# akashsengupta1997/STRAPS-3DHumanShapePose

Hardware: AMD Instinct MI355X
Metric: bodies/sec (higher is better)
Workload: dtype fp32 (encoder convolutions as exact bf16x3 operand splits (six bf16 products per term); in-step SMPL blend contraction and skinning as 3-product fp16 splits (fp16x3_lbs: 22-bit operands); fp32 accumulate throughout)

## Files before the change

include/straps_hip.h:

```cpp
#ifndef STRAPS_HIP_H
#define STRAPS_HIP_H

#include <stddef.h>
#include <stdint.h>

#ifdef __cplusplus
extern "C" {
#endif

#define STRAPS_ABI_VERSION 12

#define STRAPS_OK 0
#define STRAPS_EINVAL 1
#define STRAPS_EHIP 2
#define STRAPS_EUNSUPPORTED 3

int straps_abi_version(void);
int straps_selftest_mfma_peak(const float* seed512, float* out, int blocks, int iters, void* stream);
int straps_selftest_mfma_bf16(float* out, unsigned long long* clk2, int blocks, int iters, void* stream);
int straps_selftest_mfma_bf16_dense(float* out, unsigned long long* clk2, int blocks, int iters, int data, void* stream);
const char* straps_last_error(void);
int straps_device_count(void);
int straps_wall_clock_khz(void);
int straps_set_clock_accumulator(unsigned long long* acc2);
// ... 187 lines not shown
                         int cin, int cout, int kh, int kw, int stride, int pad, int tile_cfg, void* stream);
int straps_conv_dgrad_x3(const unsigned short* dy3, long long dy_plane_stride,
                         const unsigned short* w3_crsk, long long w_plane_stride,
                         const float* addend, float* dx_nhwc, int batch, int h, int w, int cin,
                         int cout, int kh, int kw, int stride, int pad, int tile_cfg, void* stream);
int straps_bn_apply_x3(const float* raw, const float* scale, const float* shift, const float* residual,
                       int relu, float* y, unsigned short* y_planes, long long plane_stride,
                       long long rows, int c, void* stream);
int straps_bn_relu_maxpool_fwd_x3(const float* raw, const float* scale, const float* shift,
                                  float* y_pool, uint8_t* idx, unsigned short* y_planes,
                                  long long plane_stride, int batch, int h, int w, int c, void* stream);
int straps_bn_bwd_x3(const float* dy, const float* yact, const float* raw, const float* save_mean,
                     const float* save_invstd, const float* gamma, const float* mask_scale,
                     const float* mask_shift, float* dgamma, float* dbeta, float* draw, float* dz_out,
                     unsigned short* draw_planes, long long plane_stride, void* workspace,
                     long long rows, int c, int accumulate, void* stream);
int straps_conv_dgrad_x3_bn_blocks(int batch, int h, int w, int cin, int cout, int kh, int kw, int stride,
                                   int pad, int tile_cfg);
int straps_conv_dgrad_x3_bn(const unsigned short* dy3, long long dy_plane_stride,
                            const unsigned short* w3_crsk, long long w_plane_stride, const float* addend,
                            float* dx_nhwc, int batch, int h, int w, int cin, int cout, int kh, int kw,
                            int stride, int pad, int tile_cfg, const float* bn_raw, const float* bn_out,
                            const float* bn_mask_scale, const float* bn_mask_shift, const float* bn_mean,
                            const float* bn_invstd, double* bn_partials, void* stream);
int straps_bn_bwd_finish_x3(const float* dy, const float* yact, const float* raw, const float* save_mean,
                            const float* save_invstd, const float* gamma, const float* mask_scale,
                            const float* mask_shift, float* dgamma, float* dbeta, float* draw, float* dz_out,
                            unsigned short* draw_planes, long long plane_stride, const double* partials,
                            int nblk, void* workspace, long long rows, int c, int accumulate, void* stream);
int straps_bn_apply_bits_x3(const float* raw, const float* scale, const float* shift, const float* residual, float* y,
                            unsigned short* y_planes, long long plane_stride, unsigned* relu_bits, long long rows,
                            int c, void* stream);
int straps_bn_bwd_bits_x3(const float* dy, const unsigned* relu_bits, const float* raw, const float* save_mean,
                          const float* save_invstd, const float* gamma, float* dgamma, float* dbeta, float* draw,
                          unsigned short* draw_planes, long long plane_stride, void* workspace, long long rows, int c,
                          int accumulate, void* stream);
int straps_bn_bwd_finish_bits_x3(const float* dy, const unsigned* relu_bits, const float* raw, const float* save_mean,
                                 const float* save_invstd, const float* gamma, float* dgamma, float* dbeta, float* draw,
                                 unsigned short* draw_planes, long long plane_stride, const double* partials, int nblk,
                                 void* workspace, long long rows, int c, int accumulate, void* stream);
int straps_conv_dgrad_x3_bits(const unsigned short* dy3, long long dy_plane_stride, const unsigned short* w3_crsk,
                              long long w_plane_stride, const float* addend, float* dx_nhwc, int batch, int h, int w,
                              int cin, int cout, int kh, int kw, int stride, int pad, int tile_cfg,
                              const unsigned* addend_bits, void* stream);
int straps_conv_dgrad_x3_bn_bits(const unsigned short* dy3, long long dy_plane_stride,
                                 const unsigned short* w3_crsk, long long w_plane_stride, const float* addend,
                                 float* dx_nhwc, int batch, int h, int w, int cin, int cout, int kh, int kw,
                                 int stride, int pad, int tile_cfg, const float* bn_raw, const float* bn_out,
                                 const float* bn_mask_scale, const float* bn_mask_shift, const float* bn_mean,
                                 const float* bn_invstd, double* bn_partials, const unsigned* addend_bits,
                                 const unsigned* bn_out_bits, void* stream);
int straps_conv_wgrad_x3_on_planes(int batch, int h, int w, int cin, int cout, int kh, int kw,
                                   int stride, int pad);
int straps_conv_wgrad_x3(const float* x_nhwc, const float* dy_nhwc, const unsigned short* x3,
                         long long x_plane_stride, const unsigned short* dy3, long long dy_plane_stride,
                         float* dw_oihw, void* workspace, int batch, int h, int w, int cin, int cout,
                         int kh, int kw, int stride, int pad, int accumulate, void* stream);


size_t straps_conv_wgrad_workspace_bytes(int batch, int h, int w, int cin, int cout, int kh,
                                         int kw, int stride, int pad);
int straps_conv_wgrad(const float* x_nhwc, const float* dy_nhwc, float* dw_oihw, void* workspace,
                      int batch, int h, int w, int cin, int cout, int kh, int kw, int stride,
                      int pad, int accumulate, void* stream);
size_t straps_stem_wgrad_workspace_bytes(int batch, int cin, int h, int w);
int straps_stem_wgrad(const float* x_nchw, const float* dy_nhwc, float* dw_oihw, void* workspace,
                      const uint32_t* nzmask , int batch, int cin,
                      int h, int w, int accumulate, void* stream);
#define STRAPS_STEM_DGRAD_MAX_CIN 64
size_t straps_stem_dgrad_weight_floats(int cin);
int straps_pack_stem_dgrad_weight(const float* w_oihw, float* w_pk, int cin, void* stream);
int straps_stem_dgrad(const float* dy_nhwc, const float* w_pk, float* dx_nchw, int batch, int cin, int h, int w,
                      int accumulate, void* stream);
int straps_bn_bwd_blocks(long long rows, int c);
size_t straps_bn_bwd_workspace_bytes(long long rows, int c);
int straps_bn_bwd(const float* dy, const float* yact, const float* raw, const float* save_mean,
                  const float* save_invstd, const float* gamma, const float* mask_scale,
                  const float* mask_shift, float* dgamma, float* dbeta, float* draw, float* dz_out,
                  void* workspace, long long rows, int c, int accumulate, void* stream);
int straps_bn_relu_maxpool_fwd(const float* raw_nhwc, const float* scale, const float* shift,
                               float* y_pool_nhwc, uint8_t* idx, int batch, int h, int w, int c,
                               void* stream);
int straps_bn_bwd_pooled(const float* dy_pool_nhwc, const uint8_t* idx, const float* raw,
                         const float* save_mean, const float* save_invstd, const float* gamma,
                         const float* mask_scale, const float* mask_shift, float* dgamma, float* dbeta,
                         float* draw, void* workspace, int batch, int h, int w, int c, int accumulate,
                         void* stream);
size_t straps_stem_tiles(int batch, int in_h, int in_w);
int straps_stem_tile_activity(const uint32_t* nzmask, uint8_t* tile_active, int batch, int cin, int in_h,
                              int in_w, void* stream);
int straps_bn_bwd_pooled_sparse(const float* dy_pool_nhwc, const uint8_t* idx, const float* raw,
                                const float* save_mean, const float* save_invstd, const float* gamma,
                                const float* mask_scale, const float* mask_shift, float* dgamma,
                                float* dbeta, float* draw, void* workspace, int batch, int h, int w, int c,
                                int accumulate, const uint8_t* tile_active, void* stream);
int straps_maxpool_fwd_idx(const float* x_nhwc, float* y_nhwc, uint8_t* idx, int batch, int h,
                           int w, int c, void* stream);
int straps_maxpool_bwd(const float* dy_nhwc, const uint8_t* idx, float* dx_nhwc, int batch, int h,
                       int w, int c, void* stream);
int straps_gap_bwd(const float* dfeat, float* dx_nhwc, int batch, int hw, int c, void* stream);
int straps_masked_copy(const float* x, int ldx, const float* mask, int ldmask, float* y, int ldy,
                       int m, int n, int accumulate, void* stream);
int straps_rot6d_bwd(const float* x6, long long ld, int per_row, const float* drot, float* dx6,
                     long long ldd, long long rows, void* stream);

int straps_build_proxy_input(const float* seg, const float* joints2d, float* out_nchw, int batch,
// ... 165 lines not shown
```

straps-3dhumanshapepose_amd/csrc/backward.hip:

```cpp
#include "common.h"
#include <stdlib.h>

namespace {

struct WgradP {
    const float* x;
    const float* dy;
    float* part;
    int B, H, W, Cin, Cout, R, S, stride, pad, Ho, Wo;
    int M, rows_per_split, ct, it;
};

__device__ __attribute__((aligned(16))) float k_zero16w[4] = {0.f, 0.f, 0.f, 0.f};

template <int BCO, int BCI>
__global__ __launch_bounds__(256) void conv_wgrad_kernel(WgradP p) {
    constexpr int STG = 32 * (BCO + BCI);
    constexpr int LPD = BCO / 4, PWD = 64 / LPD, RDD = 8 / PWD;
    constexpr int LPX = BCI / 4, PWX = 64 / LPX, RDX = 8 / PWX;
    constexpr int MI = BCO / 64, NI = BCI / 64;
    extern __shared__ __attribute__((aligned(16))) float smem[];
    const int tid = threadIdx.x, lane = tid & 63, wave = tid >> 6;
    const int wave_u = __builtin_amdgcn_readfirstlane(wave);
    const int wm = wave >> 1, wn = wave & 1;
// ... 404 lines not shown
            for (int c = 0; c < NI; ++c) {
                const int c4 = wn * (BCI / 2) + c * 32 + ch16 * 16 + (tt & 3) * 4;
                fx[ks][rd][c] = px * BCI + (((c4 >> 5) ^ seg_swz<BCI>(px)) << 5) + (c4 & 31);
            }
        }
    constexpr int TA[6] = {1, 0, 2, 0, 1, 0};
    constexpr int TB[6] = {1, 2, 0, 1, 0, 0};
    constexpr int DPS = 3 * (RDD + RDX);
    static_assert(DPS * (NST - 2) <= 63, "vmcnt range");
    int stage = 0;
    for (int st = 0; st < nsteps; ++st) {
        const int ahead = nsteps - 1 - st;
        if (NST >= 4 && ahead >= 2) asm volatile("s_waitcnt vmcnt(%0)" ::"n"(DPS * (NST >= 4 ? 2 : 0)) : "memory");
        else if (NST >= 3 && ahead >= 1) asm volatile("s_waitcnt vmcnt(%0)" ::"n"(DPS * (NST >= 3 ? 1 : 0)) : "memory");
        else asm volatile("s_waitcnt vmcnt(0)" ::: "memory");
        __builtin_amdgcn_s_barrier();
        asm volatile("" ::: "memory");
        if (st + NST - 1 < nsteps) dma_step(stage == 0 ? NST - 1 : stage - 1);
        const u16* D = smem + stage * STG;
        const u16* X = D + 3 * PLD;
        stage = stage + 1 == NST ? 0 : stage + 1;
        __builtin_amdgcn_s_setprio(1);
#pragma unroll
        for (int ks = 0; ks < 2; ++ks) {
            bf16x8w av[MI][3], bv[NI][3];
#pragma unroll
            for (int pl = 0; pl < 3; ++pl) {
#pragma unroll
                for (int a = 0; a < MI; ++a) av[a][pl] = tr_frag(D + pl * PLD + fd[ks][0][a], D + pl * PLD + fd[ks][1][a]);
#pragma unroll
                for (int c = 0; c < NI; ++c) bv[c][pl] = tr_frag(X + pl * PLX + fx[ks][0][c], X + pl * PLX + fx[ks][1][c]);
            }
#pragma unroll
            for (int e = 0; e < 6; ++e)
#pragma unroll
                for (int a = 0; a < MI; ++a)
#pragma unroll
                    for (int c = 0; c < NI; ++c)
                        acc[a][c] = __builtin_amdgcn_mfma_f32_32x32x16_bf16(av[a][TA[e]], bv[c][TB[e]], acc[a][c], 0, 0, 0);
        }
        __builtin_amdgcn_s_setprio(0);
    }
    const int i = lane & 31;
    const long long RS = (long long)p.R * p.S;
    float* o = p.part + (long long)split * p.Cout * RS * p.Cin;
#pragma unroll
    for (int a = 0; a < MI; ++a)
#pragma unroll
        for (int c = 0; c < NI; ++c)
#pragma unroll
            for (int q = 0; q < 16; ++q) {
                const int co = co0 + wm * (BCO / 2) + a * 32 + mfma_row(q, lane);
                o[((long long)co * RS + tap) * p.Cin + ci0 + wn * (BCI / 2) + c * 32 + i] = acc[a][c][q];
            }
}

template <int NG, int CP, int ABL = 0>
__global__ __launch_bounds__(256 * NG) void conv_wgrad3x3_x3_kernel(Wgrad3XP p) {
    constexpr int DPX = CP, XPX = CP == 32 ? 128 : 136;
    constexpr int STAGE = 3 * (DPX + XPX) * 64;
    constexpr int DR = CP / 32, XR = (XPX + 31) / 32;
    constexpr int KSG = CP / 16 / NG;
    static_assert(CP % (16 * NG) == 0, "chunk / group mismatch");
    extern __shared__ __attribute__((aligned(16))) float smem_f[];
    u16* smem = reinterpret_cast<u16*>(smem_f);
    const int pw = p.cw + 2;
    const int npatch = (p.rpc + 2) * pw;
    const int tid = threadIdx.x, lane = tid & 63, wave = (tid >> 6) & 3;
    const int grp = NG > 1 ? __builtin_amdgcn_readfirstlane(tid >> 8) : 0;
    const int wave_u = __builtin_amdgcn_readfirstlane(wave);
    const int wm = wave >> 1, wn = wave & 1;
    const int itile = blockIdx.x % p.it, ctile = blockIdx.x / p.it;
    const int co0 = ctile * 64, ci0 = itile * 64;
    const int cbeg = blockIdx.y * p.chunks_per_split;
    const int cend = min(cbeg + p.chunks_per_split, p.nchunks);
    const u16* zsrc = reinterpret_cast<const u16*>(k_zero16x);
    asm volatile("" : "+s"(zsrc));

    const int lp = (tid & 255) >> 3, ls = tid & 7;
    const int d_g = ls ^ (((lp >> 1) & 1) << 2);
    long long d_off[DR];
#pragma unroll
    for (int q = 0; q < DR; ++q) {
        const int px = lp + 32 * q;
        d_off[q] = ((long long)((co0 >> 5) + (d_g >> 2)) * p.rows + (px >> p.cw_log2) * p.W + (px & (p.cw - 1))) * 32 + (d_g & 3) * 8;
    }
    int x_pr[XR], x_pc[XR];
    long long x_g[XR];
#pragma unroll
    for (int q = 0; q < XR; ++q) {
        const int pp = lp + 32 * q;
        x_pr[q] = pp / pw - 1;
        x_pc[q] = pp - (x_pr[q] + 1) * pw - 1;
        const int g = ls ^ (((pp >> 1) & 1) << 2);
        x_g[q] = (long long)((ci0 >> 5) + (g >> 2)) * p.rows * 32 + (g & 3) * 8;
    }
    auto dma_chunk = [&](int c, int stage) {
        const int per_img = p.chunk_rows_per_img * p.chunks_per_row;
        const int b = c / per_img;
        const int rem = c - b * per_img;
        const int cr = rem / p.chunks_per_row, cc = rem - cr * p.chunks_per_row;
        const int ho0 = cr * p.rpc, wo0 = cc * p.cw;
        u16* D = smem + stage * STAGE;
        u16* X = D + 3 * DPX * 64;
        const u16* dbase = p.dy3 + ((long long)(b * p.H + ho0) * p.W + wo0) * 32;
        const u16* xsrc = p.x3 + ((long long)(b * p.H + ho0) * p.W + wo0) * 32;
// ... 951 lines not shown
    p.M = (int)M;
    const bool big = wgrad_big_tile(M, cin, cout, kh * kw);
    const int tile = big ? 128 : 64;
    p.ct = cout / tile; p.it = cin / tile;
    const int tiles = kh * kw * p.ct * p.it;
    const int splits = wgrad_splits(M, tiles, big);
    p.rows_per_split = (int)(((M + splits - 1) / splits + 31) / 32 * 32);
    hipStream_t st = (hipStream_t)stream;
    if (big) {
        STRAPS_RAISE_LDS((conv_wgrad_kernel<128, 128>), 64 * 1024, "conv_wgrad_kernel");
        hipLaunchKernelGGL((conv_wgrad_kernel<128, 128>), dim3(tiles, splits), dim3(256), 64 * 1024, st, p);
    } else {
        hipLaunchKernelGGL((conv_wgrad_kernel<64, 64>), dim3(tiles, splits), dim3(256), 32 * 1024, st, p);
    }
    STRAPS_CHECK_LAUNCH("conv_wgrad_kernel");
    const long long n = (long long)cout * kh * kw * cin;
    hipLaunchKernelGGL(wgrad_reduce_kernel, dim3((unsigned)(n / 256)), dim3(256), 0, st, p.part, dw_oihw, splits, cout, cin, kh * kw, accumulate);
    STRAPS_CHECK_LAUNCH("wgrad_reduce_kernel");
    return STRAPS_OK;
}

static int stem_wgrad_blocks(int ntiles) {
    static const int cap = STRAPS_TOOL_ENV_INT("STRAPS_STEM_WGRAD_BLOCKS", 256);
    return ntiles < cap ? ntiles : cap;
}

static int wgrad_x3_route(int batch, int h, int w, int cin, int cout, int kh, int kw, int stride, int pad) {
    Wgrad3P p3;
    int splits3;
    if (wgrad3_plan(batch, h, w, cin, cout, kh, kw, stride, pad, &p3, &splits3)) return 1;
    static const bool tap_x3 = !STRAPS_TOOL_ENV_INT("STRAPS_WGRAD_TAP_FP32", 0);
    return tap_x3 && (kh * kw > 1 || (cin >= 128 && cout >= 128)) ? 2 : 0;
}

static void wgrad_x3_block(long long M, int cin, int cout, int taps, bool big, int stride, int* bco, int* bci) {
    const int v = STRAPS_TOOL_ENV_INT("STRAPS_WGRAD_TILE", 0);
    if (v) {
        const int o = v / 1000, i = v % 1000;
        const bool known = (o == 256 && i == 64) || (o == 64 && i == 256) || (o == 256 && i == 128) || (o == 128 && i == 256) || (o == 128 && i == 64) ||
                           (o == 64 && i == 128) || (o == 128 && i == 128) || (o == 64 && i == 64);
        if (known && cout % o == 0 && cin % i == 0 && !(o == 128 && i == 128 && !big)) { *bco = o; *bci = i; }
        return;
    }
    if (taps == 1) {
        if (M >= 32768 && cout % 256 == 0 && cin % 128 == 0) { *bco = 256; *bci = 128; }
        else if (M <= 8192 && cout % 128 == 0 && cin % 128 == 0) {
            if (stride == 1 && cout > cin) { *bco = 64; *bci = 128; }
            else { *bco = 128; *bci = 64; }
        }
    } else if (cout % 256 == 0 && cin % 128 == 0) { *bco = 256; *bci = 128; }
    else if (cout % 128 == 0 && cin % 64 == 0) { *bco = 128; *bci = 64; }
}

extern "C" int straps_conv_wgrad_x3_on_planes(int batch, int h, int w, int cin, int cout, int kh, int kw, int stride, int pad) {
    return wgrad_x3_route(batch, h, w, cin, cout, kh, kw, stride, pad) != 0;
}

extern "C" int straps_conv_wgrad_x3(const float* x, const float* dy, const unsigned short* x3, long long x_plane_stride, const unsigned short* dy3,
                                    long long dy_plane_stride, float* dw_oihw, void* workspace, int batch, int h, int w, int cin, int cout, int kh,
                                    int kw, int stride, int pad, int accumulate, void* stream) {
    STRAPS_REQUIRE(dw_oihw && workspace, "straps_conv_wgrad_x3: null pointer");
    const int route = (x3 && dy3) ? wgrad_x3_route(batch, h, w, cin, cout, kh, kw, stride, pad) : 0;
    STRAPS_REQUIRE(route != 0 || (x && dy), "straps_conv_wgrad_x3: this shape runs on the fp32 tensors, which are NULL (see straps_conv_wgrad_x3_on_planes)");
    STRAPS_REQUIRE(cin % 64 == 0 && cout % 64 == 0, "straps_conv_wgrad_x3: need cin%%64==0 and cout%%64==0 (cin=%d cout=%d)", cin, cout);
    Wgrad3P p3;
    int splits3;
    if (route == 1 && wgrad3_plan(batch, h, w, cin, cout, kh, kw, stride, pad, &p3, &splits3)) {
        STRAPS_REQUIRE(x_plane_stride % 8 == 0 && dy_plane_stride % 8 == 0, "straps_conv_wgrad_x3: plane strides must be multiples of 8 elements");
        Wgrad3XP q;
        q.x3 = x3; q.dy3 = dy3; q.xps = x_plane_stride; q.dps = dy_plane_stride; q.part = (float*)workspace;
        q.H = p3.H; q.W = p3.W; q.Cin = p3.Cin; q.Cout = p3.Cout; q.cw = p3.cw; q.cw_log2 = p3.cw_log2; q.rpc = p3.rpc;
        q.chunks_per_row = p3.chunks_per_row; q.chunk_rows_per_img = p3.chunk_rows_per_img; q.nchunks = p3.nchunks;
        q.chunks_per_split = p3.chunks_per_split; q.it = p3.it;
        q.rows = (long long)batch * h * w;
        constexpr int W3X_NG = 2;
        hipStream_t st3 = (hipStream_t)stream;
        Wgrad3P p64;
        int splits64;
        const bool c64 = wgrad3_plan(batch, h, w, cin, cout, kh, kw, stride, pad, &p64, &splits64, 64) && splits64 <= splits3;
        if (c64) {
            q.rpc = p64.rpc; q.chunks_per_row = p64.chunks_per_row; q.chunk_rows_per_img = p64.chunk_rows_per_img; q.nchunks = p64.nchunks;
            q.chunks_per_split = p64.chunks_per_split;
            splits3 = splits64;
            const size_t lds = (size_t)2 * 3 * (64 + 136) * 64 * sizeof(u16);
            const dim3 grid3((cout / 64) * (cin / 64), splits3);
#ifdef STRAPS_TOOLS
            static const int abl = STRAPS_TOOL_ENV_INT("STRAPS_WGRAD3_ABL", 0);
            if (abl) {
                auto kern = abl == 1 ? conv_wgrad3x3_x3_kernel<W3X_NG, 64, 1> : abl == 2 ? conv_wgrad3x3_x3_kernel<W3X_NG, 64, 2>
                          : abl == 3 ? conv_wgrad3x3_x3_kernel<W3X_NG, 64, 3> : abl == 4 ? conv_wgrad3x3_x3_kernel<W3X_NG, 64, 4> : conv_wgrad3x3_x3_kernel<W3X_NG, 64, 5>;
                hipFuncSetAttribute((const void*)kern, hipFuncAttributeMaxDynamicSharedMemorySize, (int)lds);
                hipLaunchKernelGGL(kern, grid3, dim3(256 * W3X_NG), lds, st3, q);
                STRAPS_CHECK_LAUNCH("conv_wgrad3x3_x3_kernel (ablation)");
                return STRAPS_OK;
            }
#endif
            STRAPS_RAISE_LDS((conv_wgrad3x3_x3_kernel<W3X_NG, 64>), lds, "conv_wgrad3x3_x3_kernel");
            hipLaunchKernelGGL((conv_wgrad3x3_x3_kernel<W3X_NG, 64>), grid3, dim3(256 * W3X_NG), lds, st3, q);
        } else {
            const size_t lds = (size_t)2 * 3 * (32 + 128) * 64 * sizeof(u16);
            STRAPS_RAISE_LDS((conv_wgrad3x3_x3_kernel<W3X_NG, 32>), lds, "conv_wgrad3x3_x3_kernel");
            hipLaunchKernelGGL((conv_wgrad3x3_x3_kernel<W3X_NG, 32>), dim3((cout / 64) * (cin / 64), splits3), dim3(256 * W3X_NG), lds, st3, q);
        }
        STRAPS_CHECK_LAUNCH("conv_wgrad3x3_x3_kernel");
        const long long n3 = (long long)cout * 9 * cin;
        hipLaunchKernelGGL(wgrad_reduce_kernel, dim3((unsigned)(n3 / 256)), dim3(256), 0, st3, q.part, dw_oihw, splits3, cout, cin, 9, accumulate);
        STRAPS_CHECK_LAUNCH("wgrad_reduce_kernel");
        return STRAPS_OK;
    }
    if (route == 2) {
        STRAPS_REQUIRE(x_plane_stride % 8 == 0 && dy_plane_stride % 8 == 0, "straps_conv_wgrad_x3: plane strides must be multiples of 8 elements");
        WgradXP q;
        q.x3 = x3; q.dy3 = dy3; q.xps = x_plane_stride; q.dps = dy_plane_stride; q.part = (float*)workspace;
        q.B = batch; q.H = h; q.W = w; q.Cin = cin; q.Cout = cout; q.R = kh; q.S = kw; q.stride = stride; q.pad = pad;
        q.Ho = (h + 2 * pad - kh) / stride + 1;
        q.Wo = (w + 2 * pad - kw) / stride + 1;
        const long long M = (long long)batch * q.Ho * q.Wo;
        STRAPS_REQUIRE(M < (1LL << 31), "straps_conv_wgrad_x3: problem too large");
        q.M = (int)M;
        const bool big = wgrad_big_tile(M, cin, cout, kh * kw);
        int bco = big ? 128 : 64, bci = bco;
        wgrad_x3_block(M, cin, cout, kh * kw, big, stride, &bco, &bci);
        q.ct = cout / bco; q.it = cin / bci;
        const int tiles = kh * kw * q.ct * q.it;
        const size_t lds = (size_t)2 * 3 * 32 * (bco + bci) * sizeof(u16);
        int splits;
        if (bco == bci) splits = wgrad_splits(M, tiles, bco == 128, true);
        else {
            const int per_cu = (int)((160 * 1024) / lds) < 1 ? 1 : (int)((160 * 1024) / lds);
            splits = (256 * per_cu + tiles - 1) / tiles;
            const long long max_s = (M + 127) / 128;
            if (splits > max_s) splits = (int)max_s;
            const int cap = wgrad_splits(M, kh * kw * (cout / (big ? 128 : 64)) * (cin / (big ? 128 : 64)), big);
            if (splits > cap) splits = cap;
            if (splits < 1) splits = 1;
        }
        q.rows_per_split = (int)(((M + splits - 1) / splits + 31) / 32 * 32);
        hipStream_t st = (hipStream_t)stream;
        static const int nst_env = STRAPS_TOOL_ENV_INT("STRAPS_WGRAD_TAP_NST", 2);
        constexpr int SB = 3 * 32 * 256 * 2, SS = 3 * 32 * 128 * 2;
#define STRAPS_WGRAD_X3_LAUNCH(BCO_, BCI_)                                                                              \
        do {                                                                                                            \
            STRAPS_RAISE_LDS((conv_wgrad_x3_kernel<BCO_, BCI_, 2>), lds, "conv_wgrad_x3_kernel");                       \
            hipLaunchKernelGGL((conv_wgrad_x3_kernel<BCO_, BCI_, 2>), dim3(tiles, splits), dim3(256), lds, st, q);      \
        } while (0)
        if (bco == 256 && bci == 64) STRAPS_WGRAD_X3_LAUNCH(256, 64);
        else if (bco == 64 && bci == 256) STRAPS_WGRAD_X3_LAUNCH(64, 256);
        else if (bco == 256 && bci == 128) STRAPS_WGRAD_X3_LAUNCH(256, 128);
        else if (bco == 128 && bci == 256) STRAPS_WGRAD_X3_LAUNCH(128, 256);
        else if (bco == 128 && bci == 64) STRAPS_WGRAD_X3_LAUNCH(128, 64);
        else if (bco == 64 && bci == 128) STRAPS_WGRAD_X3_LAUNCH(64, 128);
        else if (bco == 128) {
            if (nst_env == 3) {
                STRAPS_RAISE_LDS((conv_wgrad_x3_kernel<128, 128, 3>), 3 * SB, "conv_wgrad_x3_kernel");
                hipLaunchKernelGGL((conv_wgrad_x3_kernel<128, 128, 3>), dim3(tiles, splits), dim3(256), 3 * SB, st, q);
            } else {
                STRAPS_RAISE_LDS((conv_wgrad_x3_kernel<128, 128, 2>), 2 * SB, "conv_wgrad_x3_kernel");
                hipLaunchKernelGGL((conv_wgrad_x3_kernel<128, 128, 2>), dim3(tiles, splits), dim3(256), 2 * SB, st, q);
            }
        } else if (nst_env == 3) {
            STRAPS_RAISE_LDS((conv_wgrad_x3_kernel<64, 64, 3>), 3 * SS, "conv_wgrad_x3_kernel");
            hipLaunchKernelGGL((conv_wgrad_x3_kernel<64, 64, 3>), dim3(tiles, splits), dim3(256), 3 * SS, st, q);
        } else if (nst_env == 4) {
            STRAPS_RAISE_LDS((conv_wgrad_x3_kernel<64, 64, 4>), 4 * SS, "conv_wgrad_x3_kernel");
            hipLaunchKernelGGL((conv_wgrad_x3_kernel<64, 64, 4>), dim3(tiles, splits), dim3(256), 4 * SS, st, q);
        } else {
            hipLaunchKernelGGL((conv_wgrad_x3_kernel<64, 64, 2>), dim3(tiles, splits), dim3(256), 2 * SS, st, q);
        }
#undef STRAPS_WGRAD_X3_LAUNCH
        STRAPS_CHECK_LAUNCH("conv_wgrad_x3_kernel");
        const long long n = (long long)cout * kh * kw * cin;
        hipLaunchKernelGGL(wgrad_reduce_kernel, dim3((unsigned)(n / 256)), dim3(256), 0, st, q.part, dw_oihw, splits, cout, cin, kh * kw, accumulate);
        STRAPS_CHECK_LAUNCH("wgrad_reduce_kernel");
        return STRAPS_OK;
    }
    return straps_conv_wgrad(x, dy, dw_oihw, workspace, batch, h, w, cin, cout, kh, kw, stride, pad, accumulate, stream);
}

extern "C" size_t straps_stem_wgrad_workspace_bytes(int batch, int cin, int h, int w) {
    const int Ho = (h - 1) / 2 + 1, Wo = (w - 1) / 2 + 1;
    const int ntiles = batch * ((Ho + TY - 1) / TY) * ((Wo + TX - 1) / TX);
    const int Kp = (cin * 49 + 31) / 32 * 32;
    const size_t groups = (cin + CG - 1) / CG;
    return (size_t)stem_wgrad_blocks(ntiles) * 64 * Kp * sizeof(float) + straps_stem_nzmask_words(batch, cin, h, w) * sizeof(uint32_t) +
           ((groups * ntiles + 3) & ~(size_t)3);
}

extern "C" int straps_stem_wgrad(const float* x_nchw, const float* dy_nhwc, float* dw_oihw, void* workspace, const uint32_t* nzmask,
                                 int batch, int cin, int h, int w, int accumulate, void* stream) {
    STRAPS_REQUIRE(x_nchw && dy_nhwc && dw_oihw && workspace, "straps_stem_wgrad: null pointer");
    STRAPS_REQUIRE(batch > 0 && cin > 0 && h >= 7 && w >= 7, "straps_stem_wgrad: bad shape B=%d C=%d H=%d W=%d", batch, cin, h, w);
    const int K = cin * 49, Kp = (K + 31) / 32 * 32;
    const int Ho = (h - 1) / 2 + 1, Wo = (w - 1) / 2 + 1;
    const int tiles_x = (Wo + TX - 1) / TX, tiles_y = (Ho + TY - 1) / TY;
    const int ntiles = batch * tiles_x * tiles_y;
    const int nblk = stem_wgrad_blocks(ntiles);
    const int groups = (cin + CG - 1) / CG;
    STRAPS_REQUIRE(groups <= 65535, "straps_stem_wgrad: too many input channels (%d)", cin);
    hipStream_t st = (hipStream_t)stream;
// ... 249 lines not shown
```

straps-3dhumanshapepose_amd/hipabi.py:

```python
import ctypes as C
import os
import subprocess

_HERE = os.path.dirname(os.path.abspath(__file__))
CSRC = os.path.join(_HERE, 'csrc')
LIB_PATH = os.path.join(CSRC, 'libstraps_hip.so')
HEADER = os.path.join(os.path.dirname(_HERE), 'include', 'straps_hip.h')
SOURCES = ['abi.hip', 'augment.hip', 'pose.hip', 'ief.hip', 'elementwise.hip', 'conv.hip', 'conv_x3.hip', 'conv_x3_lean.hip', 'conv_bf16.hip', 'conv_x3f.hip', 'conv_wgrad_x3f.hip', 'stem.hip', 'stem_dgrad.hip', 'smpl.hip',
           'smpl_bwd.hip', 'backward.hip', 'train.hip', 'metrics.hip', 'image.hip', 'raster.hip', 'exchange.hip',
           'regressor.hip', 'regressor_train.hip', 'predict.hip', 'eval.hip', 'fit.hip', 'silfit.hip', 'render.hip']

_lib = None
LINK_LIBS = ['-ldl']
EXTRA_FLAGS = {'smpl.hip': ['-fno-slp-vectorize']}


def _existing_sources():
    return [os.path.join(CSRC, s) for s in SOURCES if os.path.isfile(os.path.join(CSRC, s))]


TOOLS_LIB_PATH = os.path.join(os.path.dirname(_HERE), 'tools', 'bin', 'libstraps_hip_tools.so')


def build(force=False, verbose=False, tools=False):
# ... 106 lines not shown
    _fields_ = [('wh', C.c_int32), ('lattice', C.c_int32), ('tau', C.c_float), ('w_in', C.c_float), ('w_out', C.c_float)]


class RenderOptsStruct(C.Structure):
    _fields_ = [('colour', C.c_float * 3), ('ambient', C.c_float), ('background', C.c_float * 3), ('n_lights', C.c_int32), ('light_dir', C.c_float * 12),
                ('light_intensity', C.c_float * 4)]


_P, _I, _L, _F, _Z, _D = C.c_void_p, C.c_int, C.c_longlong, C.c_float, C.c_size_t, C.c_double

ABI_VERSION = 12
SIGNATURES = {
    'straps_abi_version': (_I, []),
    'straps_last_error': (C.c_char_p, []),
    'straps_device_count': (_I, []),
    'straps_wall_clock_khz': (_I, []),
    'straps_set_clock_accumulator': (_I, [_P]),
    'straps_selftest_mfma_peak': (_I, [_P, _P, _I, _I, _P]),
    'straps_selftest_mfma_bf16': (_I, [_P, _P, _I, _I, _P]),
    'straps_selftest_mfma_bf16_dense': (_I, [_P, _P, _I, _I, _I, _P]),
    'straps_pack_conv_weight': (_I, [_P, _P, _I, _I, _I, _I, _P]),
    'straps_pack_conv_weight_dgrad': (_I, [_P, _P, _I, _I, _I, _I, _P]),
    'straps_pack_conv_weights_batched': (_I, [_P, _I, _L, _P]),
    'straps_pack_conv_weights_batched_x3': (_I, [_P, _I, _L, _P, _P, _L, _P]),
    'straps_stem_weight_floats': (_Z, [_I]),
    'straps_pack_stem_weight': (_I, [_P, _P, _I, _P]),
    'straps_bn_fold': (_I, [_P, _P, _P, _P, _F, _P, _P, _I, _P]),
    'straps_bn_fold_stats': (_I, [_P, _P, _P, _P, _F, _P, _P, _P, _P, _I, _P]),
    'straps_stem_stat_blocks': (_I, [_I, _I, _I]),
    'straps_stem_nzmask_words': (_Z, [_I, _I, _I, _I]),
    'straps_stem_nzmask': (_I, [_P, _P, _I, _I, _I, _I, _P]),
    'straps_stem_fwd': (_I, [_P, _P, _P, _P, _I, _P, _P, _P, _I, _I, _I, _I, _P]),
    'straps_conv_trace_buffer': (_I, [_P]),
    'straps_split3_bf16': (_I, [_P, _P, _L, _L, _P]),
    'straps_split3_bf16_cm': (_I, [_P, _P, _L, _I, _L, _P]),
    'straps_conv_fwd_x3': (_I, [_P, _L, _P, _L, _P, _P, _P, _I, _P, _P, _I, _I, _I, _I, _I, _I, _I, _I, _I, _I, _P]),
    'straps_conv_fwd_x3p': (_I, [_P, _L, _P, _L, _P, _P, _P, _I, _P, _P, _L, _I, _I, _I, _I, _I, _I, _I, _I, _I, _I, _P]),
    'straps_conv_dgrad_x3': (_I, [_P, _L, _P, _L, _P, _P, _I, _I, _I, _I, _I, _I, _I, _I, _I, _I, _P]),
    'straps_split_bf16_cm': (_I, [_P, _P, _L, _I, _P]),
    'straps_pack_conv_weight_bf16': (_I, [_P, _P, _I, _I, _I, _I, _P]),
    'straps_conv_bf16_tile_choice': (_I, [_I] * 9),
    'straps_conv_fwd_bf16': (_I, [_P, _P, _P, _P, _P, _I, _P, _P] + [_I] * 10 + [_P]),
    'straps_conv_x3_stat_blocks': (_I, [_I] * 10),
    'straps_conv_x3f_supported': (_I, [_I] * 6),
    'straps_conv_fwd_x3f': (_I, [_P, _P, _P, _I, _P, _L, _P, _P, _P, _I, _P, _P] + [_I] * 10 + [_P]),
    'straps_conv_x3f_stat_blocks': (_I, [_I] * 10),
    'straps_conv_dgrad_x3f': (_I, [_P, _P, _L, _P, _P, _P] + [_I] * 10 + [_P] * 8),
    'straps_conv_dgrad_x3f_bn_blocks': (_I, [_I] * 10),
    'straps_conv_wgrad_x3f_workspace_bytes': (_Z, [_I] * 9),
    'straps_conv_wgrad_x3f': (_I, [_P, _P, _P, _I, _P, _P, _P] + [_I] * 10 + [_P]),
    'straps_bn_apply_x3': (_I, [_P, _P, _P, _P, _I, _P, _P, _L, _L, _I, _P]),
    'straps_bn_relu_maxpool_fwd_x3': (_I, [_P, _P, _P, _P, _P, _P, _L, _I, _I, _I, _I, _P]),
    'straps_conv_wgrad_x3_on_planes': (_I, [_I] * 9),
    'straps_conv_dgrad_x3_bn_blocks': (_I, [_I] * 10),
    'straps_conv_dgrad_x3_bn': (_I, [_P, _L, _P, _L, _P, _P, _I, _I, _I, _I, _I, _I, _I, _I, _I, _I, _P, _P, _P, _P, _P, _P, _P, _P]),
    'straps_bn_bwd_finish_x3': (_I, [_P] * 13 + [_L, _P, _I, _P, _L, _I, _I, _P]),
    'straps_conv_wgrad_x3': (_I, [_P, _P, _P, _L, _P, _L, _P, _P, _I, _I, _I, _I, _I, _I, _I, _I, _I, _I, _P]),
    'straps_bn_bwd_x3': (_I, [_P] * 13 + [_L, _P, _L, _I, _I, _P]),
    'straps_bn_apply_bits_x3': (_I, [_P, _P, _P, _P, _P, _P, _L, _P, _L, _I, _P]),
    'straps_bn_bwd_bits_x3': (_I, [_P] * 10 + [_L, _P, _L, _I, _I, _P]),
    'straps_bn_bwd_finish_bits_x3': (_I, [_P] * 10 + [_L, _P, _I, _P, _L, _I, _I, _P]),
    'straps_conv_dgrad_x3_bits': (_I, [_P, _L, _P, _L, _P, _P, _I, _I, _I, _I, _I, _I, _I, _I, _I, _I, _P, _P]),
    'straps_conv_dgrad_x3_bn_bits': (_I, [_P, _L, _P, _L, _P, _P, _I, _I, _I, _I, _I, _I, _I, _I, _I, _I, _P, _P, _P, _P, _P, _P, _P, _P, _P, _P]),
    'straps_conv_stat_blocks': (_I, [_I, _I, _I, _I, _I, _I]),
    'straps_conv_fwd': (_I, [_P, _P, _P, _P, _P, _I, _P, _P, _I, _I, _I, _I, _I, _I, _I, _I, _I, _I, _P]),
    'straps_maxpool_fwd': (_I, [_P, _P, _I, _I, _I, _I, _P]),
    'straps_gap_fwd': (_I, [_P, _P, _I, _I, _I, _P]),
    'straps_bn_stats_finalize': (_I, [_P, _I, _I, _L, _P, _P, _F, _F, _P, _P, _P, _P, _P, _P, _P]),
    'straps_bn_apply': (_I, [_P, _P, _P, _P, _I, _P, _L, _I, _P]),
    'straps_linear_fwd': (_I, [_P, _I, _P, _I, _P, _P, _P, _I, _I, _I, _I, _I, _P]),
    'straps_broadcast_rows': (_I, [_P, _I, _P, _I, _I, _P]),
    'straps_ief_pack': (_I, [_P, _P, _P, _P, _P, _I, _I, _I, _I, _I, _P]),
    'straps_gemm_multi': (_I, [C.POINTER(GemmDesc), _I, _P]),
    'straps_rot6d_fwd': (_I, [_P, _L, _I, _P, _L, _P]),
    'straps_rodrigues_fwd': (_I, [_P, _P, _L, _P]),
    'straps_rodrigues_bwd': (_I, [_P, _P, _P, _L, _P]),
    'straps_orthographic_project': (_I, [_P, _P, _I, _P, _L, _I, _P]),
    'straps_orthographic_project_bwd': (_I, [_P, _P, _I, _P, _P, _P, _L, _I, _P]),
    'straps_perspective_project': (_I, [_P, _P, _P, _P, _I, _P, _L, _I, _P]),
    'straps_smpl_workspace_bytes': (_Z, [C.POINTER(SmplModelStruct), _L]),
    'straps_smpl_fwd': (_I, [C.POINTER(SmplModelStruct), _P, _P, _P, _P, _P, _L, _I, _I, _P]),
    'straps_smpl_bwd_workspace_bytes': (_Z, [_L, _I]),
    'straps_smpl_bwd': (_I, [C.POINTER(SmplModelStruct), _P, _P, _P, _P, _P, _P, _P, _L, _I, _P]),
    'straps_smpl_bwd_aa': (_I, [C.POINTER(SmplModelStruct), _P, _P, _P, _P, _P, _P, _P, _P, _P, _L, _I, _P]),
    'straps_conv_dgrad': (_I, [_P, _P, _P, _P, _I, _I, _I, _I, _I, _I, _I, _I, _I, _I, _P]),
    'straps_conv_wgrad_workspace_bytes': (_Z, [_I, _I, _I, _I, _I, _I, _I, _I, _I]),
    'straps_conv_wgrad': (_I, [_P, _P, _P, _P, _I, _I, _I, _I, _I, _I, _I, _I, _I, _I, _P]),
    'straps_stem_wgrad_workspace_bytes': (_Z, [_I, _I, _I, _I]),
    'straps_stem_wgrad': (_I, [_P, _P, _P, _P, _P, _I, _I, _I, _I, _I, _P]),
    'straps_stem_dgrad_weight_floats': (_Z, [_I]),
    'straps_pack_stem_dgrad_weight': (_I, [_P, _P, _I, _P]),
    'straps_stem_dgrad': (_I, [_P, _P, _P, _I, _I, _I, _I, _I, _P]),
    'straps_bn_bwd_blocks': (_I, [_L, _I]),
    'straps_bn_bwd_workspace_bytes': (_Z, [_L, _I]),
    'straps_bn_bwd': (_I, [_P, _P, _P, _P, _P, _P, _P, _P, _P, _P, _P, _P, _P, _L, _I, _I, _P]),
    'straps_bn_relu_maxpool_fwd': (_I, [_P, _P, _P, _P, _P, _I, _I, _I, _I, _P]),
    'straps_bn_bwd_pooled': (_I, [_P, _P, _P, _P, _P, _P, _P, _P, _P, _P, _P, _P, _I, _I, _I, _I, _I, _P]),
    'straps_bn_bwd_pooled_sparse': (_I, [_P, _P, _P, _P, _P, _P, _P, _P, _P, _P, _P, _P, _I, _I, _I, _I, _I, _P, _P]),
    'straps_stem_tiles': (_Z, [_I, _I, _I]),
    'straps_stem_tile_activity': (_I, [_P, _P, _I, _I, _I, _I, _P]),
    'straps_maxpool_fwd_idx': (_I, [_P, _P, _P, _I, _I, _I, _I, _P]),
    'straps_maxpool_bwd': (_I, [_P, _P, _P, _I, _I, _I, _I, _P]),
    'straps_gap_bwd': (_I, [_P, _P, _I, _I, _I, _P]),
    'straps_masked_copy': (_I, [_P, _I, _P, _I, _P, _I, _I, _I, _I, _P]),
    'straps_rot6d_bwd': (_I, [_P, _L, _I, _P, _P, _L, _L, _P]),
    'straps_build_proxy_input': (_I, [_P, _P, _P, _I, _I, _I, _P]),
# ... 161 lines not shown
```

Baseline: 7977.

## Add row-wise wgrad kernel computing three kernel columns per block for stride-2 3x3

Adds a weight-gradient kernel for 3x3 stride-2 pad-1 convolutions that assigns one kernel row per block and computes all three column taps at once. It stages even and odd input pixel columns of the row in LDS so the dy tile is loaded once and reused across three taps. This is meant to cut redundant dy loads and the block count relative to the per-tap kernel. It raises LDS use (one block per CU) and accumulator registers, applies only when Wo is 8, 16 or 32 with a 128x64 tile, and is gated by an env var that defaults to on. A launch-shape query entry point and a shared planning helper are also added.

```diff
diff --git a/include/straps_hip.h b/include/straps_hip.h
--- a/include/straps_hip.h
+++ b/include/straps_hip.h
@@ -263,6 +263,8 @@
                                  const unsigned* bn_out_bits, void* stream);
 int straps_conv_wgrad_x3_on_planes(int batch, int h, int w, int cin, int cout, int kh, int kw,
                                    int stride, int pad);
+int straps_conv_wgrad_x3_launch_shape(int batch, int h, int w, int cin, int cout, int kh, int kw,
+                                      int stride, int pad, int* workgroups, int* slots);
 int straps_conv_wgrad_x3(const float* x_nhwc, const float* dy_nhwc, const unsigned short* x3,
                          long long x_plane_stride, const unsigned short* dy3, long long dy_plane_stride,
                          float* dw_oihw, void* workspace, int batch, int h, int w, int cin, int cout,
diff --git a/straps-3dhumanshapepose_amd/csrc/backward.hip b/straps-3dhumanshapepose_amd/csrc/backward.hip
--- a/straps-3dhumanshapepose_amd/csrc/backward.hip
+++ b/straps-3dhumanshapepose_amd/csrc/backward.hip
@@ -480,6 +480,174 @@
             for (int q = 0; q < 16; ++q) {
                 const int co = co0 + wm * (BCO / 2) + a * 32 + mfma_row(q, lane);
                 o[((long long)co * RS + tap) * p.Cin + ci0 + wn * (BCI / 2) + c * 32 + i] = acc[a][c][q];
+            }
+}
+
+constexpr int WROW_XO = 40;
+template <int BCO, int BCI>
+__global__ __launch_bounds__(256) void conv_wgrad_x3_row_kernel(WgradXP p, int lg_wo) {
+    constexpr int NST = 2;
+    static_assert(BCI == 64, "eight lanes per pixel row, eight rows per wave copy");
+    constexpr int PLD = 32 * BCO, PLE = 32 * BCI, PLO = WROW_XO * BCI;
+    constexpr int STG = 3 * (PLD + PLE + PLO);
+    constexpr int LPD = BCO / 8, PWD = 64 / LPD, RDD = 8 / PWD;
+    constexpr int MI = BCO / 64;
+    extern __shared__ __attribute__((aligned(16))) float smem_f[];
+    u16* smem = reinterpret_cast<u16*>(smem_f);
+    const int tid = threadIdx.x, lane = tid & 63, wave = tid >> 6;
+    const int wave_u = __builtin_amdgcn_readfirstlane(wave);
+    const int wm = wave >> 1, wn = wave & 1;
+    int t = blockIdx.x;
+    const int itile = t % p.it; t /= p.it;
+    const int ctile = t % p.ct; t /= p.ct;
+    const int r = t;
+    const int split = blockIdx.y;
+    const int co0 = ctile * BCO, ci0 = itile * BCI;
+    const int mbeg = split * p.rows_per_split;
+    const int mend = min(mbeg + p.rows_per_split, p.M);
+    const int nsteps = mend > mbeg ? (mend - mbeg + 31) >> 5 : 0;
+    const int Wo = 1 << lg_wo, nr = 32 >> lg_wo;
+    const int row_end = mend >> lg_wo;
+    const u16* zsrc = reinterpret_cast<const u16*>(k_zero16w);
+    asm volatile("" : "+s"(zsrc));
+
+    int md[RDD];
+    long long gd[RDD];
+    const long long xrows = (long long)p.B * p.H * p.W;
+#pragma unroll
+    for (int q = 0; q < RDD; ++q) {
+        const int px = (q * 4 + wave) * PWD + lane / LPD, j = lane % LPD;
+        md[q] = mbeg + px;
+        const int c = co0 + ((((j >> 2) ^ seg_swz<BCO>(px)) << 2) | (j & 3)) * 8;
+        gd[q] = (long long)(c >> 5) * p.M * 32 + (c & 31);
+    }
+    int xrow[3], xwi[3];
+    long long gx[3];
+    bool xok[3];
+    int row0 = mbeg >> lg_wo;
+#pragma unroll
+    for (int q = 0; q < 3; ++q) {
+        const int slot = (q == 2 ? 32 : wave * 8) + (lane >> 3), j = lane & 7;
+        const int c = ci0 + ((((j >> 2) ^ seg_swz<BCI>(slot)) << 2) | (j & 3)) * 8;
+        gx[q] = (long long)(c >> 5) * xrows * 32 + (c & 31);
+        if (q == 0) {
+            xrow[q] = slot >> lg_wo;
+            xwi[q] = 2 * (slot & (Wo - 1));
+            xok[q] = true;
+        } else {
+            xrow[q] = slot / (Wo + 1);
+            xwi[q] = 2 * (slot - xrow[q] * (Wo + 1)) - 1;
+            xok[q] = xrow[q] < nr && xwi[q] >= 0;
+        }
+        xok[q] = xok[q] && xwi[q] < p.W;
+    }
+    auto dma_step = [&](int stage) {
+        u16* D = smem + stage * STG;
+        u16* XE = D + 3 * PLD;
+        u16* XO = XE + 3 * PLE;
+#pragma unroll
+        for (int q = 0; q < RDD; ++q) {
+            const bool in = md[q] < mend;
+            const u16* src = in ? p.dy3 + (long long)md[q] * 32 + gd[q] : zsrc;
+            const long long ps = in ? p.dps : 0;
+            md[q] += 32;
+#pragma unroll
+            for (int pl = 0; pl < 3; ++pl)
+                __builtin_amdgcn_global_load_lds((const __attribute__((address_space(1))) void*)(src + pl * ps),
+                                                 (__attribute__((address_space(3))) void*)(D + pl * PLD + (q * 4 + wave_u) * PWD * BCO), 16, 0, 0);
+        }
+#pragma unroll
+        for (int q = 0; q < 3; ++q) {
+            if (q == 2 && wave_u != 0) break;
+            const int row = row0 + xrow[q];
+            const int b = row / p.Ho, ho = row - b * p.Ho;
+            const int hi = ho * 2 - 1 + r;
+            const bool in = xok[q] && row < row_end && (unsigned)hi < (unsigned)p.H;
+            const u16* src = in ? p.x3 + (((long long)b * p.H + hi) * p.W + xwi[q]) * 32 + gx[q] : zsrc;
+            const long long ps = in ? p.xps : 0;
+            u16* dst = q == 0 ? XE + wave_u * 8 * BCI : XO + (q == 2 ? 32 : wave_u * 8) * BCI;
+            const int pls = q == 0 ? PLE : PLO;
+#pragma unroll
+            for (int pl = 0; pl < 3; ++pl)
+                __builtin_amdgcn_global_load_lds((const __attribute__((address_space(1))) void*)(src + pl * ps),
+                                                 (__attribute__((address_space(3))) void*)(dst + pl * pls), 16, 0, 0);
+        }
+        row0 += nr;
+    };
+    f32x16 acc[3][MI];
+#pragma unroll
+    for (int s = 0; s < 3; ++s)
+#pragma unroll
+        for (int a = 0; a < MI; ++a)
+#pragma unroll
+            for (int q = 0; q < 16; ++q) acc[s][a][q] = 0.f;
+#pragma unroll
+    for (int s0 = 0; s0 < NST - 1; ++s0)
+        if (s0 < nsteps) dma_step(s0);
+    const int tt = lane & 15, ch16 = (lane >> 4) & 1, kh = lane >> 5;
+    int fd[2][2][MI], fx[3][2][2];
+#pragma unroll
+    for (int ks = 0; ks < 2; ++ks)
+#pragma unroll
+        for (int rd = 0; rd < 2; ++rd) {
+            const int px = ks * 16 + kh * 8 + rd * 4 + (tt >> 2);
+#pragma unroll
+            for (int a = 0; a < MI; ++a) {
+                const int c4 = wm * (BCO / 2) + a * 32 + ch16 * 16 + (tt & 3) * 4;
+                fd[ks][rd][a] = px * BCO + (((c4 >> 5) ^ seg_swz<BCO>(px)) << 5) + (c4 & 31);
+            }
+            const int c4 = wn * (BCI / 2) + ch16 * 16 + (tt & 3) * 4;
+#pragma unroll
+            for (int s = 0; s < 3; ++s) {
+                const int slot = s == 1 ? px : px + (px >> lg_wo) + (s >> 1);
+                fx[s][ks][rd] = (s == 1 ? 0 : 3 * PLE) + slot * BCI + (((c4 >> 5) ^ seg_swz<BCI>(slot)) << 5) + (c4 & 31);
+            }
+        }
+    constexpr int TA[6] = {1, 0, 2, 0, 1, 0};
+    constexpr int TB[6] = {1, 2, 0, 1, 0, 0};
+    int stage = 0;
+    for (int st = 0; st < nsteps; ++st) {
+        asm volatile("s_waitcnt vmcnt(0)" ::: "memory");
+        __builtin_amdgcn_s_barrier();
+        asm volatile("" ::: "memory");
+        if (st + NST - 1 < nsteps) dma_step(stage == 0 ? NST - 1 : stage - 1);
+        const u16* D = smem + stage * STG;
+        const u16* X = D + 3 * PLD;
+        stage = stage + 1 == NST ? 0 : stage + 1;
+        __builtin_amdgcn_s_setprio(1);
+#pragma unroll
+        for (int ks = 0; ks < 2; ++ks) {
+            bf16x8w av[MI][3], bv[3][3];
+#pragma unroll
+            for (int pl = 0; pl < 3; ++pl) {
+#pragma unroll
+                for (int a = 0; a < MI; ++a) av[a][pl] = tr_frag(D + pl * PLD + fd[ks][0][a], D + pl * PLD + fd[ks][1][a]);
+#pragma unroll
+                for (int s = 0; s < 3; ++s) {
+                    const int po = pl * (s == 1 ? PLE : PLO);
+                    bv[s][pl] = tr_frag(X + po + fx[s][ks][0], X + po + fx[s][ks][1]);
+                }
+            }
+#pragma unroll
+            for (int e = 0; e < 6; ++e)
+#pragma unroll
+                for (int s = 0; s < 3; ++s)
+#pragma unroll
+                    for (int a = 0; a < MI; ++a)
+                        acc[s][a] = __builtin_amdgcn_mfma_f32_32x32x16_bf16(av[a][TA[e]], bv[s][TB[e]], acc[s][a], 0, 0, 0);
+        }
+        __builtin_amdgcn_s_setprio(0);
+    }
+    const int i = lane & 31;
+    float* o = p.part + (long long)split * p.Cout * 9 * p.Cin;
+#pragma unroll
+    for (int s = 0; s < 3; ++s)
+#pragma unroll
+        for (int a = 0; a < MI; ++a)
+#pragma unroll
+            for (int q = 0; q < 16; ++q) {
+                const int co = co0 + wm * (BCO / 2) + a * 32 + mfma_row(q, lane);
+                o[((long long)co * 9 + r * 3 + s) * p.Cin + ci0 + wn * (BCI / 2) + i] = acc[s][a][q];
             }
 }
 
@@ -1537,8 +1705,72 @@
     else if (cout % 128 == 0 && cin % 64 == 0) { *bco = 128; *bci = 64; }
 }
 
+struct WgradTapPlan {
+    int bco, bci, tiles, splits, per_cu;
+    size_t lds;
+    bool row;
+};
+
+static WgradTapPlan wgrad_x3_tap_plan(long long M, int cin, int cout, int kh, int kw, int stride, int pad, int wo) {
+    WgradTapPlan t;
+    const int taps = kh * kw;
+    const bool big = wgrad_big_tile(M, cin, cout, taps);
+    t.bco = big ? 128 : 64; t.bci = t.bco;
+    wgrad_x3_block(M, cin, cout, taps, big, stride, &t.bco, &t.bci);
+    t.row = false;
+    t.tiles = taps * (cout / t.bco) * (cin / t.bci);
+    t.lds = (size_t)2 * 3 * 32 * (t.bco + t.bci) * sizeof(u16);
+    const int by_lds = (int)((160 * 1024) / t.lds);
+    t.per_cu = by_lds < 1 ? 1 : by_lds > 8 ? 8 : by_lds;
+    if (t.bco == t.bci) t.splits = wgrad_splits(M, t.tiles, t.bco == 128, true);
+    else {
+        int splits = (256 * (by_lds < 1 ? 1 : by_lds) + t.tiles - 1) / t.tiles;
+        const long long max_s = (M + 127) / 128;
+        if (splits > max_s) splits = (int)max_s;
+        const int cap = wgrad_splits(M, taps * (cout / (big ? 128 : 64)) * (cin / (big ? 128 : 64)), big);
+        if (splits > cap) splits = cap;
+        t.splits = splits < 1 ? 1 : splits;
+    }
+    const int row_tiles = 3 * (cout / t.bco) * (cin / t.bci);
+    if (kh == 3 && kw == 3 && stride == 2 && pad == 1 && t.bco == 128 && t.bci == 64 && (wo == 8 || wo == 16 || wo == 32) && row_tiles * t.splits <= 256 &&
+        STRAPS_TOOL_ENV_INT("STRAPS_WGRAD_ROW", 1)) {
+        t.row = true;
+        t.tiles = row_tiles;
+        t.lds = (size_t)2 * 3 * (32 * t.bco + (32 + WROW_XO) * t.bci) * sizeof(u16);
+        t.per_cu = 1;
+    }
+    return t;
+}
+
 extern "C" int straps_conv_wgrad_x3_on_planes(int batch, int h, int w, int cin, int cout, int kh, int kw, int stride, int pad) {
     return wgrad_x3_route(batch, h, w, cin, cout, kh, kw, stride, pad) != 0;
+}
+
+extern "C" int straps_conv_wgrad_x3_launch_shape(int batch, int h, int w, int cin, int cout, int kh, int kw, int stride, int pad, int* workgroups,
+                                                 int* slots) {
+    STRAPS_REQUIRE(workgroups && slots, "straps_conv_wgrad_x3_launch_shape: null pointer");
+    STRAPS_REQUIRE(batch > 0 && h > 0 && w > 0 && kh > 0 && kw > 0 && stride > 0 && pad >= 0 && h + 2 * pad >= kh && w + 2 * pad >= kw,
+                   "straps_conv_wgrad_x3_launch_shape: bad shape B=%d H=%d W=%d k=%dx%d stride=%d pad=%d", batch, h, w, kh, kw, stride, pad);
+    STRAPS_REQUIRE(cin > 0 && cout > 0 && cin % 64 == 0 && cout % 64 == 0,
+                   "straps_conv_wgrad_x3_launch_shape: need cin%%64==0 and cout%%64==0 (cin=%d cout=%d)", cin, cout);
+    const int route = wgrad_x3_route(batch, h, w, cin, cout, kh, kw, stride, pad);
+    STRAPS_REQUIRE(route != 0, "straps_conv_wgrad_x3_launch_shape: this shape runs on the fp32 tensors (see straps_conv_wgrad_x3_on_planes)");
+    if (route == 1) {
+        Wgrad3P p3, p64;
+        int splits3 = 0, splits64 = 0;
+        wgrad3_plan(batch, h, w, cin, cout, kh, kw, stride, pad, &p3, &splits3);
+        if (wgrad3_plan(batch, h, w, cin, cout, kh, kw, stride, pad, &p64, &splits64, 64) && splits64 <= splits3) splits3 = splits64;
+        *workgroups = (cout / 64) * (cin / 64) * splits3;
+        *slots = 256;
+        return STRAPS_OK;
+    }
+    const int ho = (h + 2 * pad - kh) / stride + 1, wo = (w + 2 * pad - kw) / stride + 1;
+    const long long M = (long long)batch * ho * wo;
+    STRAPS_REQUIRE(M < (1LL << 31), "straps_conv_wgrad_x3_launch_shape: problem too large");
+    const WgradTapPlan t = wgrad_x3_tap_plan(M, cin, cout, kh, kw, stride, pad, wo);
+    *workgroups = t.tiles * t.splits;
+    *slots = 256 * t.per_cu;
+    return STRAPS_OK;
 }
 
 extern "C" int straps_conv_wgrad_x3(const float* x, const float* dy, const unsigned short* x3, long long x_plane_stride, const unsigned short* dy3,
@@ -1603,23 +1835,10 @@
         const long long M = (long long)batch * q.Ho * q.Wo;
         STRAPS_REQUIRE(M < (1LL << 31), "straps_conv_wgrad_x3: problem too large");
         q.M = (int)M;
-        const bool big = wgrad_big_tile(M, cin, cout, kh * kw);
-        int bco = big ? 128 : 64, bci = bco;
-        wgrad_x3_block(M, cin, cout, kh * kw, big, stride, &bco, &bci);
+        const WgradTapPlan plan = wgrad_x3_tap_plan(M, cin, cout, kh, kw, stride, pad, q.Wo);
+        const int bco = plan.bco, bci = plan.bci, tiles = plan.tiles, splits = plan.splits;
+        const size_t lds = plan.lds;
         q.ct = cout / bco; q.it = cin / bci;
-        const int tiles = kh * kw * q.ct * q.it;
-        const size_t lds = (size_t)2 * 3 * 32 * (bco + bci) * sizeof(u16);
-        int splits;
-        if (bco == bci) splits = wgrad_splits(M, tiles, bco == 128, true);
-        else {
-            const int per_cu = (int)((160 * 1024) / lds) < 1 ? 1 : (int)((160 * 1024) / lds);
-            splits = (256 * per_cu + tiles - 1) / tiles;
-            const long long max_s = (M + 127) / 128;
-            if (splits > max_s) splits = (int)max_s;
-            const int cap = wgrad_splits(M, kh * kw * (cout / (big ? 128 : 64)) * (cin / (big ? 128 : 64)), big);
-            if (splits > cap) splits = cap;
-            if (splits < 1) splits = 1;
-        }
         q.rows_per_split = (int)(((M + splits - 1) / splits + 31) / 32 * 32);
         hipStream_t st = (hipStream_t)stream;
         static const int nst_env = STRAPS_TOOL_ENV_INT("STRAPS_WGRAD_TAP_NST", 2);
@@ -1629,7 +1848,10 @@
             STRAPS_RAISE_LDS((conv_wgrad_x3_kernel<BCO_, BCI_, 2>), lds, "conv_wgrad_x3_kernel");                       \
             hipLaunchKernelGGL((conv_wgrad_x3_kernel<BCO_, BCI_, 2>), dim3(tiles, splits), dim3(256), lds, st, q);      \
         } while (0)
-        if (bco == 256 && bci == 64) STRAPS_WGRAD_X3_LAUNCH(256, 64);
+        if (plan.row) {
+            STRAPS_RAISE_LDS((conv_wgrad_x3_row_kernel<128, 64>), lds, "conv_wgrad_x3_row_kernel");
+            hipLaunchKernelGGL((conv_wgrad_x3_row_kernel<128, 64>), dim3(tiles, splits), dim3(256), lds, st, q, q.Wo == 8 ? 3 : q.Wo == 16 ? 4 : 5);
+        } else if (bco == 256 && bci == 64) STRAPS_WGRAD_X3_LAUNCH(256, 64);
         else if (bco == 64 && bci == 256) STRAPS_WGRAD_X3_LAUNCH(64, 256);
         else if (bco == 256 && bci == 128) STRAPS_WGRAD_X3_LAUNCH(256, 128);
         else if (bco == 128 && bci == 256) STRAPS_WGRAD_X3_LAUNCH(128, 256);
diff --git a/straps-3dhumanshapepose_amd/hipabi.py b/straps-3dhumanshapepose_amd/hipabi.py
--- a/straps-3dhumanshapepose_amd/hipabi.py
+++ b/straps-3dhumanshapepose_amd/hipabi.py
@@ -182,6 +182,7 @@
     'straps_bn_apply_x3': (_I, [_P, _P, _P, _P, _I, _P, _P, _L, _L, _I, _P]),
     'straps_bn_relu_maxpool_fwd_x3': (_I, [_P, _P, _P, _P, _P, _P, _L, _I, _I, _I, _I, _P]),
     'straps_conv_wgrad_x3_on_planes': (_I, [_I] * 9),
+    'straps_conv_wgrad_x3_launch_shape': (_I, [_I] * 9 + [_P, _P]),
     'straps_conv_dgrad_x3_bn_blocks': (_I, [_I] * 10),
     'straps_conv_dgrad_x3_bn': (_I, [_P, _L, _P, _L, _P, _P, _I, _I, _I, _I, _I, _I, _I, _I, _I, _I, _P, _P, _P, _P, _P, _P, _P, _P]),
     'straps_bn_bwd_finish_x3': (_I, [_P] * 13 + [_L, _P, _I, _P, _L, _I, _I, _P]),
```

Result: no change. 8007 (median of 6 runs) (+0.4%).
